# elizabethfong/SparkSmithWaterman

Hardware: NVIDIA B200
Metric: GCUPS incl. traceback (150 bp reads x 10k RefSeq-shaped refs per B200) (higher is better)
Workload: dtype s16x2

## Files before the change

### sparksmithwaterman_b200/csrc/swb_align.cu

```cuda
#include "swb_host.h"

using namespace swbh;

namespace {
struct Segments { std::vector<int32_t> ref, c0, len, skip, end; };
void make_segments(const swb_refset *rs, int K, int match, int mismatch, int gap, bool few_items, Segments &S)
{
    const int64_t m = (int64_t)GL * K;
    const int64_t big = std::max({match, mismatch, 0});
    const int64_t W = m + (big * m) / (-(int64_t)gap) + 1;
    const int64_t W_al = ((W + 8 + 15) / 16) * 16;
    int64_t SEG = few_items ? 1024 : 8192;
    SEG = std::max<int64_t>(SEG, ((2 * W_al + 15) / 16) * 16);
    const int32_t BIG = 1 << 26;
    struct One { int32_t ref, c0, len, skip, end; };
    std::vector<One> v;
    v.reserve((size_t)rs->n_refs + 64);
    for (int64_t s = 0; s < rs->n_refs; ++s) {
        const int64_t n = rs->len_sorted[(size_t)s];
        if (n <= 2 * SEG) { v.push_back(One{(int32_t)s, 0, (int32_t)n, 0, BIG}); continue; }
        const int64_t nseg = (n + SEG - 1) / SEG;
        for (int64_t k = 0; k < nseg; ++k) {
            const int64_t lo = k * SEG, hi = std::min<int64_t>(n, (k + 1) * SEG);
            const int64_t c0 = std::max<int64_t>(0, lo - W_al);
            v.push_back(One{(int32_t)s, (int32_t)c0, (int32_t)(hi - c0), (int32_t)((lo - c0) / CB),
                            k == nseg - 1 ? BIG : (int32_t)((hi - c0) / CB)});
        }
    }
    std::stable_sort(v.begin(), v.end(), [](const One &a, const One &b) { return a.len > b.len; });
    S.ref.clear(); S.c0.clear(); S.len.clear(); S.skip.clear(); S.end.clear();
    for (const One &o : v) { S.ref.push_back(o.ref); S.c0.push_back(o.c0); S.len.push_back(o.len); S.skip.push_back(o.skip); S.end.push_back(o.end); }
}

int pick_k(int m)
{
    for (int k = 0; k < kNumK; ++k)
        if (GL * kKList[k] >= m) return kKList[k];
    return 0;
}

int record_words(int K) { return ((K + 1 + 7) / 8 + CB / 8) * 8; }

using ResultPtr = std::unique_ptr<swb_result, void (*)(swb_result *)>;
ResultPtr new_result(swb_ctx *ctx, const swb_refset *rs, const swb_reads *rd, uint32_t flags)
{
    ResultPtr res(new swb_result(), swb_result_free);
    ctx->live.fetch_add(1);
    res->ctx = ctx; res->n_refs = rs->n_refs; res->n_reads = rd->n_reads; res->flags = flags;
    res->ref_len = rs->len_orig; res->read_len = rd->len;
    int64_t read_bases = 0;
    for (int32_t m : rd->len) read_bases += m;
    res->stats[STAT_CELLS] = (double)rs->total_bases * (double)read_bases;
    res->stats[STAT_PAIRS] = (double)rs->n_refs * (double)rd->n_reads;
    return res;
}
}

struct AlignCall::Batch {
    int n_rp = 0, m_max = 0;
    std::vector<int32_t> h_rp;
    BatchParams P;
};

int AlignCall::run(int32_t *ext_scores, int32_t *ext_totals)
{
    const int64_t n_refs = rs->n_refs, n_reads = rd->n_reads;
    const size_t n_pairs = (size_t)(n_refs * n_reads);
    if (ext_scores) res->d_scores.view(ext_scores, n_pairs); else CU(res->d_scores.alloc(n_pairs, st));
    if (ext_totals) res->d_totals.view(ext_totals, (size_t)n_refs); else CU(res->d_totals.alloc((size_t)n_refs, st));
    CU(res->d_best.alloc((size_t)n_reads * 4, st));
    CU(cudaMemsetAsync(res->d_scores.p, 0, std::max<size_t>(n_pairs, 1) * 4, st));
    res->top_k = top_k; res->min_score = min_score;
    if (top_k > 0) CU(res->d_hits.alloc((size_t)n_reads * top_k * 4, st));

    const auto t_wall0 = std::chrono::steady_clock::now();
    ctx->ev_used = 0;
    CU(ctx->counters.reserve(16, st));
    int rc;
    if (n_refs > 0 && n_reads > 0) {
        std::vector<std::vector<int32_t>> classes(kNumK);
        std::vector<int32_t> wide;
        classify_reads(classes, wide);
        for (int kc = 0; kc < kNumK; ++kc)
            if (!classes[(size_t)kc].empty() && (rc = run_class(kKList[kc], classes[(size_t)kc]))) return rc;
        if (!wide.empty() && (rc = run_wide_reads(wide))) return rc;
    }
    DevBuf<uint32_t> keep;
    if (top_k > 0 && (rc = select_final_hits(keep))) return rc;
    if ((rc = assemble(keep))) return rc;
    return finish_stats(t_wall0);
}

void AlignCall::classify_reads(std::vector<std::vector<int32_t>> &classes, std::vector<int32_t> &wide) const
{
    const bool short_scores_ok = rs->two_bit_ok && gap < 0 && std::abs((int64_t)match) <= 8000 &&
                                 std::abs((int64_t)mismatch) <= 8000 && std::abs((int64_t)gap) <= 8000;
    static const bool no_long = getenv("SWB_NO_LONG_CLASSES") != nullptr;
    const bool long_kernels_ok = !no_long && tile_trace_ok(match, mismatch, gap);
    for (int64_t q = 0; q < rd->n_reads; ++q) {
        const int m = rd->len[(size_t)q];
        if (m == 0) continue;
        const int64_t smax = (int64_t)std::max({match, mismatch, 0}) * std::min<int64_t>(m, rs->max_len);
        const bool is_short = short_scores_ok && smax <= 16000 &&
                              (m <= MAX_SHORT_ROWS || (m <= MAX_LONG_ROWS && long_kernels_ok && fill_bias_ok(match, mismatch, gap, smax)));
        if (!is_short) { wide.push_back((int32_t)q); continue; }
        const int K = pick_k(m);
        for (int k = 0; k < kNumK; ++k) if (kKList[k] == K) classes[(size_t)k].push_back((int32_t)q);
    }
}

int AlignCall::run_class(int K, std::vector<int32_t> &reads)
{
    std::stable_sort(reads.begin(), reads.end(), [&](int32_t a, int32_t b) { return rd->len[(size_t)a] > rd->len[(size_t)b]; });
    const int64_t n_rp_total = ((int64_t)reads.size() + 1) / 2;
    std::shared_ptr<swb_refset::SegTables> segt;
    int rc = seg_tables(K, n_rp_total * ((rs->n_refs + 3) / 4) < (int64_t)ctx->sm_count * 24, segt);
    if (rc) return rc;
    const int64_t bytes_per_rp = rs->blocks_per_rp * ((int64_t)record_words(K) * GL * 4 + GL * 4);
    int64_t rp_per_batch = std::max<int64_t>(1, ctx->ws_bytes / std::max<int64_t>(bytes_per_rp, 1));
    rp_per_batch = std::min<int64_t>(rp_per_batch, 1 << 16);
    if (rp_per_batch * rs->n_refs * 2 >= ((int64_t)1 << 30)) rp_per_batch = std::max<int64_t>(1, (((int64_t)1 << 30) - 1) / (rs->n_refs * 2));
    const int64_t nb = (n_rp_total + rp_per_batch - 1) / rp_per_batch;
    rp_per_batch = (n_rp_total + nb - 1) / nb;
    std::vector<Batch> batches((size_t)nb);
    for (int64_t k = 0; k < nb; ++k) {
        const int64_t rp0 = k * rp_per_batch;
        Batch &b = batches[(size_t)k];
        if ((rc = fill_batch(K, reads, rp0, (int)std::min<int64_t>(rp_per_batch, n_rp_total - rp0), *segt, b))) return rc;
        if ((rc = trace_batch(K, b))) return rc;
    }
    CU(cudaStreamSynchronize(st));
    return SWB_OK;
}

int AlignCall::seg_tables(int K, bool few_items, std::shared_ptr<swb_refset::SegTables> &out)
{
    const swb_refset::SegKey skey{K, match, mismatch, gap, few_items ? 1 : 0};
    auto sit = rs->seg_cache.find(skey);
    if (sit == rs->seg_cache.end()) {
        Segments segs;
        make_segments(rs, K, match, mismatch, gap, few_items, segs);
        auto sc = std::make_shared<swb_refset::SegTables>();
        sc->nv = segs.ref.size();
        CU(sc->ref.alloc(sc->nv, st)); CU(sc->c0.alloc(sc->nv, st)); CU(sc->len.alloc(sc->nv, st));
        CU(sc->skip.alloc(sc->nv, st)); CU(sc->end.alloc(sc->nv, st));
        CU(cudaMemcpyAsync(sc->ref.p, segs.ref.data(), sc->nv * 4, cudaMemcpyHostToDevice, st));
        CU(cudaMemcpyAsync(sc->c0.p, segs.c0.data(), sc->nv * 4, cudaMemcpyHostToDevice, st));
        CU(cudaMemcpyAsync(sc->len.p, segs.len.data(), sc->nv * 4, cudaMemcpyHostToDevice, st));
        CU(cudaMemcpyAsync(sc->skip.p, segs.skip.data(), sc->nv * 4, cudaMemcpyHostToDevice, st));
        CU(cudaMemcpyAsync(sc->end.p, segs.end.data(), sc->nv * 4, cudaMemcpyHostToDevice, st));
        CU(cudaStreamSynchronize(st));
        if (rs->seg_cache.size() >= 16) rs->seg_cache.clear();
        sit = rs->seg_cache.emplace(skey, sc).first;
    }
    out = sit->second;
    return SWB_OK;
}

int AlignCall::fill_batch(int K, const std::vector<int32_t> &reads, int64_t rp0, int n_rp, const swb_refset::SegTables &segt, Batch &b)
{
    b.n_rp = n_rp;
    b.h_rp.assign((size_t)n_rp * 2, -1);
    for (int r = 0; r < n_rp; ++r)
        for (int h = 0; h < 2; ++h) {
            const int64_t x = (rp0 + r) * 2 + h;
            if (x < (int64_t)reads.size()) {
                b.h_rp[(size_t)r * 2 + h] = reads[(size_t)x];
                b.m_max = std::max(b.m_max, rd->len[(size_t)reads[(size_t)x]]);
            }
        }
    ++n_batches;
    CU(ctx->rp.reserve(b.h_rp.size(), st));
    CU(cudaMemcpyAsync(ctx->rp.p, b.h_rp.data(), b.h_rp.size() * 4, cudaMemcpyHostToDevice, st));
    const size_t ck_words = (size_t)n_rp * rs->blocks_per_rp * record_words(K) * GL;
    const size_t tmx_words = (size_t)n_rp * rs->blocks_per_rp * GL;
    CU(ctx->ck.reserve(ck_words, st));
    CU(ctx->tmx.reserve(tmx_words, st));
    ck_bytes += (double)(ck_words + tmx_words) * 4;
    BatchParams &P = b.P;
    P.ref_words = rs->words.p; P.ref_word_off = rs->word_off.p; P.ref_len = rs->len.p;
    P.ref_orig = rs->orig.p; P.ref_sorted_of = rs->sorted_of.p; P.ref_blk_off = rs->blk_off.p;
    P.n_refs = (int32_t)rs->n_refs; P.blocks_per_rp = rs->blocks_per_rp;
    P.v_ref = segt.ref.p; P.v_c0 = segt.c0.p; P.v_len = segt.len.p; P.v_skip = segt.skip.p;
    P.v_end = segt.end.p; P.n_vrefs = (int32_t)segt.nv;
    P.read_codes = rd->codes.p; P.read_off = rd->off.p; P.rp_reads = ctx->rp.p; P.read_slot = nullptr;
    P.n_rp = n_rp; P.n_reads = rd->n_reads;
    P.match = match; P.mismatch = mismatch; P.gap = gap; P.tie_gt = (flags & SWB_F_TIE_GT) ? 1 : 0;
    P.scores = res->d_scores.p; P.rec = ctx->ck.p; P.tmx = ctx->tmx.p; P.sel = nullptr;
    uint32_t *d_work = ctx->counters.p + 4;
    const bool biased = fill_bias_ok(match, mismatch, gap, (int64_t)std::max({match, mismatch, 0}) * std::min<int64_t>(b.m_max, rs->max_len));
    P.seam_bias = biased ? -gap : 0;
    P.tmx_slack = biased ? fill_sub_slack(match, mismatch, gap) : 0;
    CU(timer.begin(STAT_FILL_MS));
    if (biased)
        CU(launch_fill_bias(K, P, d_work, ctx->sm_count, st));
    else
        CU(launch_fill(K, P, d_work, ctx->sm_count, st));
    ++launches;
    CU(timer.end());
    return SWB_OK;
}

int AlignCall::trace_batch(int K, Batch &b)
{
    const bool scores_only = (flags & SWB_F_SCORES_ONLY) != 0;
    size_t sel_words = 0;
    if (top_k > 0 && !scores_only) {
        sel_words = ((size_t)b.n_rp * 2 * (size_t)rs->n_refs + 31) / 32;
        CU(ctx->hit_sel.reserve(sel_words, st));
        b.P.sel = ctx->hit_sel.p;
    }
    const BatchParams &P = b.P;
    if (scores_only && P.tmx_slack == 0) return SWB_OK;
    CU(timer.begin(STAT_LOCATE_MS));
    uint32_t n_cells = 0;
    const int rc = locate_cells(K, b, sel_words, n_cells);
    if (rc) return rc;
    if (scores_only) { CU(timer.end()); return SWB_OK; }
    BatchOut bo;
    bo.n_cells = n_cells;
    CU(bo.keys.alloc(n_cells, st));
    const size_t tmp_bytes = sort_keys_tmp_bytes(n_cells);
    CU(ctx->sort_tmp.reserve(tmp_bytes, st));
    CU(sort_keys(ctx->keys_tmp.p, bo.keys.p, n_cells, ctx->sort_tmp.p, tmp_bytes, st));
    launches += 4;
    CU(timer.end());

    CU(timer.begin(STAT_TRACE_MS));
    const int64_t big = std::max({match, mismatch, 0});
    int64_t lmax = (int64_t)b.m_max + (big * b.m_max - 1) / (-(int64_t)gap) + 1;
    lmax = std::min<int64_t>(lmax, (int64_t)b.m_max + rs->max_len);
    bo.ops_stride = (int)((lmax + 15) / 16);
    CU(bo.beg.alloc(n_cells, st));
    CU(bo.oplen.alloc(n_cells, st));
    CU(bo.ops.alloc((size_t)n_cells * bo.ops_stride, st));
    if (tile_trace_ok(match, mismatch, gap))
        CU(launch_tile_trace(K, P, bo.keys.p, n_cells, bo.beg.p, bo.oplen.p, bo.ops.p, (int)bo.ops_stride, ctx->sm_count, st));
    else
        CU(launch_trace(K, P, bo.keys.p, n_cells, bo.beg.p, bo.oplen.p, bo.ops.p, (int)bo.ops_stride, ctx->sm_count, st));
    ++launches;
    CU(timer.end());
    res->stats[STAT_MAX_CELLS] += n_cells;
    CU(bo.d_slot_read.alloc(b.h_rp.size(), st));
    CU(cudaMemcpyAsync(bo.d_slot_read.p, b.h_rp.data(), b.h_rp.size() * 4, cudaMemcpyHostToDevice, st));
    res->batches.push_back(std::move(bo));
    return SWB_OK;
}

int AlignCall::locate_cells(int K, const Batch &b, size_t sel_words, uint32_t &n_cells)
{
    const BatchParams &P = b.P;
    const bool scores_only = (flags & SWB_F_SCORES_ONLY) != 0;
    uint32_t *d_ntasks = ctx->counters.p, *d_ncells = ctx->counters.p + 1;
    const int64_t pairs_b = (int64_t)b.n_rp * 2 * rs->n_refs;
    uint32_t cap_tasks = (uint32_t)std::min<int64_t>(pairs_b * (P.tmx_slack > 0 ? 4 : 2) + 1024, (int64_t)1 << 31);
    uint32_t cap_cells = (uint32_t)std::min<int64_t>(pairs_b * 2 + 4096, (int64_t)1 << 31);
    uint32_t h_counts[2] = {0, 0};
    for (int attempt = 0; attempt < 3; ++attempt) {
        CU(ctx->tasks.reserve(cap_tasks, st));
        CU(ctx->task_hits.reserve((size_t)cap_tasks * locate_hit_bytes(), st));
        CU(ctx->keys_tmp.reserve(cap_cells, st));
        CU(cudaMemsetAsync(ctx->counters.p, 0, 8, st));
        CU(launch_flag_tiles(P, ctx->tasks.p, cap_tasks, d_ntasks, ctx->sm_count, st));
        CU(launch_locate(K, P, ctx->tasks.p, d_ntasks, cap_tasks, ctx->task_hits.p, ctx->keys_tmp.p, cap_cells, d_ncells,
                         ctx->sm_count, 0, st));
        launches += 2;
        if (sel_words) {
            CU(timer.begin(STAT_SELECT_MS));
            CU(cudaMemsetAsync(ctx->hit_sel.p, 0, sel_words * 4, st));
// ... 458 lines not shown
```

### sparksmithwaterman_b200/csrc/swb_fill_bias.cu

```cuda
#include "swb_internal.h"
#include "swb_device.cuh"

#include <algorithm>
#include <cstdlib>

namespace swb {

__device__ __forceinline__ uint32_t imad_add(uint32_t a, uint32_t one, uint32_t b)
{
    return a * one + b;
}

template <int K>
__device__ __forceinline__ void fill_column(uint32_t (&H)[K], const uint32_t *pcol, uint32_t diag, uint32_t top,
                                            uint32_t floorv, uint32_t g2, uint32_t one)
{
    using G = Geo<K>;
    uint32_t nw = diag, nn = top;
    if constexpr (K <= MAX_K_BASE) {
        uint32_t sv[G::KP];
        load_profile<G::KP>(pcol, sv);
#pragma unroll
        for (int r = 0; r < K; ++r) {
            const uint32_t tt = imad_add(nw, one, sv[r]);
            const uint32_t pre = vmax3(tt, H[r], floorv);
            nw = H[r];
            H[r] = viaddmax(nn, g2, pre);
            nn = H[r];
        }
    } else {
        const uint4 *p4 = reinterpret_cast<const uint4 *>(pcol);
#pragma unroll
        for (int q = 0; q < G::KP / 4; ++q) {
            const uint4 v = p4[q];
            const uint32_t sv[4] = {v.x, v.y, v.z, v.w};
#pragma unroll
            for (int x = 0; x < 4; ++x) {
                const int r = 4 * q + x;
                if (r < K) {
                    const uint32_t tt = imad_add(nw, one, sv[x]);
                    const uint32_t pre = vmax3(tt, H[r < K ? r : 0], floorv);
                    nw = H[r < K ? r : 0];
                    H[r < K ? r : 0] = viaddmax(nn, g2, pre);
                    nn = H[r < K ? r : 0];
                }
            }
        }
    }
}

constexpr int FILL_ROLL_K = 25;
constexpr int fill_bias_threads(int K) { return K <= MAX_K_BASE ? 512 : (K <= 48 ? 384 : 256); }

template <int K, bool SUB>
__global__ void __launch_bounds__(fill_bias_threads(K)) fill_bias_kernel(const BatchParams P, uint32_t *work_counter, uint32_t one)
{
    using G = Geo<K>;
    extern __shared__ __align__(16) uint32_t prof_all[];

    const int lane = threadIdx.x & 31, warp = threadIdx.x >> 5;
    const int t = lane & (GL - 1), g = lane >> 3;
    uint32_t *prof = prof_all + warp * G::PROF_WORDS;
    const int n_quads = (P.n_vrefs + 3) >> 2;
    const uint32_t n_items = (uint32_t)n_quads * (uint32_t)P.n_rp;

    const int ag = -P.gap;
    const uint32_t g2 = pack2(P.gap, P.gap);
    const uint32_t gpos = pack2(ag, ag);
    const uint32_t base_bias = pack2(ag * (8 - t), ag * (8 - t));
    const uint32_t renorm = (uint32_t)(-(int32_t)(pack2(ag * CB, ag * CB)));
    const uint32_t unbias = (uint32_t)(-(int32_t)base_bias);
    const uint32_t negbase = pack2(-ag * (8 - t), -ag * (8 - t));
    const uint32_t g2c = g2 - 0x10000u, g2c2 = 2u * g2c;
    static_assert((CB & 1) == 0, "the subsampled tile maximum tracks the odd steps of a block");
    const int my_prof = t * G::KS;
    int cur_rp = -1, ra = 0, rb = -1;

    for (;;) {
        uint32_t item = 0;
        if (lane == 0) item = atomicAdd(work_counter, 1u);
        item = __shfl_sync(0xffffffffu, item, 0);
        if (item >= n_items) break;
        const int q = (int)(item / (uint32_t)P.n_rp);
        const int rp = (int)(item - (uint32_t)q * (uint32_t)P.n_rp);
        if (rp != cur_rp) {
            cur_rp = rp;
            ra = P.rp_reads[2 * rp]; rb = P.rp_reads[2 * rp + 1];
            const int64_t offa = P.read_off[ra];
            const int ma = (int)(P.read_off[ra + 1] - offa);
            const int64_t offb = rb >= 0 ? P.read_off[rb] : 0;
            const int mb = rb >= 0 ? (int)(P.read_off[rb + 1] - offb) : 0;
            __syncwarp();
            for (int idx = lane; idx < GL * K; idx += 32) {
                const int tt = idx / K, r = idx - tt * K;
                const int row = tt * K + r;
                const int qa = row < ma ? (int)P.read_codes[offa + row] : -1;
                const int qb = row < mb ? (int)P.read_codes[offb + row] : -1;
#pragma unroll
                for (int c = 0; c < 4; ++c) {
                    const int lo = qa < 0 ? 0 : (qa == c ? P.match : P.mismatch) + ag;
                    const int hi = qb < 0 ? 0 : (qb == c ? P.match : P.mismatch) + ag;
                    prof[c * G::CSTRIDE + tt * G::KS + r] = pack2(lo, hi);
                }
            }
            __syncwarp();
        }

        const int v = 4 * q + g;
        const bool has_ref = v < P.n_vrefs;
        const int ref = has_ref ? P.v_ref[v] : 0;
        const int c0 = has_ref ? P.v_c0[v] : 0;
        const int n_g = has_ref ? P.v_len[v] : 0;
        const int skip = has_ref ? P.v_skip[v] : 0;
        const int own_end = has_ref ? P.v_end[v] : 0;
        const int nmax = P.v_len[4 * q];
        const int nmin = (4 * q + 3 < P.n_vrefs) ? P.v_len[4 * q + 3] : 0;
        const uint32_t *wp = P.ref_words + (has_ref ? P.ref_word_off[ref] + (uint32_t)(c0 >> 4) : 0u);
        const int64_t blk0 = (int64_t)rp * P.blocks_per_rp + (has_ref ? P.ref_blk_off[ref] + c0 / CB : 0);
        const int my_steps = has_ref ? min(n_g + GL - 1, own_end * CB) : 0;

        uint32_t H[K];
#pragma unroll
        for (int r = 0; r < K; ++r) H[r] = base_bias;
        uint32_t diag = base_bias, floorv = base_bias, negfloor = negbase;
        uint32_t tmax = 0, gmax = 0, wprev = 0;

        const int nsteps = nmax + GL - 1;
        for (int s0 = 0; s0 < nsteps; s0 += 16) {
            const uint32_t wnew = (s0 < n_g) ? __ldg(wp + (s0 >> 4)) : 0u;
            const uint32_t win = __funnelshift_rc(wprev, wnew, 32 - 2 * t);
            wprev = wnew;
            const bool fast = (s0 >= GL - 1) && (s0 + 16 <= nmin);

            const bool own_chunk = (s0 < my_steps) && ((s0 >> 4) >= skip);
            uint32_t *seam = rec_lane<K>(P.rec, blk0 + (s0 >> 4), t) + G::CKP * REC_P;
            uint32_t tq[8] = {0, 0, 0, 0, 0, 0, 0, 0};

            if (fast) {
                constexpr int UNR = K < FILL_ROLL_K ? 16 : 8;
#pragma unroll 1
                for (int uq = 0; uq < 16; uq += UNR) {
                    const uint32_t winq = win >> (2 * uq);
#pragma unroll
                    for (int uu = 0; uu < UNR; ++uu) {
                        floorv = imad_add(floorv, one, gpos);
                        if (!SUB) negfloor = imad_add(negfloor, one, g2c);
                        uint32_t top = __shfl_up_sync(0xffffffffu, H[K - 1], 1);
                        if (t == 0) top = floorv;
                        const uint32_t c = (winq >> (2 * uu)) & 3u;
                        fill_column<K>(H, prof + c * G::CSTRIDE + my_prof, diag, top, floorv, g2, one);
                        diag = top;
                        if (!SUB) tmax = viaddmax(colmax<K>(floorv, H), negfloor, tmax);
                        else if (uu & 1) {
                            negfloor = imad_add(negfloor, one, g2c2);
                            tmax = viaddmax(colmax_even<K>(floorv, H), negfloor, tmax);
                        }
                        tq[uu & 7] = top;
                        if ((uu & 7) == 7 && own_chunk)
                            stg256(seam + ((uq + uu) >> 3) * REC_P, tq[0], tq[1], tq[2], tq[3], tq[4], tq[5], tq[6], tq[7]);
                    }
                }
            } else {
#pragma unroll 1
                for (int uq = 0; uq < 16; uq += 8) {
#pragma unroll
                    for (int uu = 0; uu < 8; ++uu) {
                        const int u = uq + uu;
                        const int s = s0 + u;
                        floorv = imad_add(floorv, one, gpos);
                        negfloor = imad_add(negfloor, one, g2c);
                        uint32_t top = __shfl_up_sync(0xffffffffu, H[K - 1], 1);
                        if (t == 0) top = floorv;
                        const uint32_t c = (win >> (2 * u)) & 3u;
                        const bool valid = (s >= t) && (s < n_g + t);
                        if (valid) {
                            fill_column<K>(H, prof + c * G::CSTRIDE + my_prof, diag, top, floorv, g2, one);
                            tmax = viaddmax(colmax<K>(floorv, H), negfloor, tmax);
                        } else {
#pragma unroll
                            for (int r = 0; r < K; ++r) H[r] = floorv;
                        }
                        diag = top;
                        tq[uu] = top;
                        if (uu == 7 && own_chunk) stg256(seam + (uq >> 3) * REC_P, tq[0], tq[1], tq[2], tq[3], tq[4], tq[5], tq[6], tq[7]);
                    }
                }
            }

            const int s_next = s0 + 16;
            {
#pragma unroll
                for (int r = 0; r < K; ++r) H[r] = imad_add(H[r], one, renorm);
                diag = imad_add(diag, one, renorm);
                floorv = base_bias;
                negfloor = negbase;
                const int b = s_next / CB;
                if (s_next - CB < my_steps && b - 1 >= skip) {
                    P.tmx[(blk0 + b - 1) * GL + t] = tmax;
                    gmax = vmax2(gmax, tmax);
                }
                tmax = 0;
                if constexpr (K <= MAX_K_BASE) {
                    uint32_t U[K];
#pragma unroll
                    for (int r = 0; r < K; ++r) U[r] = imad_add(H[r], one, unbias);
                    if (s_next < my_steps && b >= skip)
                        store_checkpoint<K>(rec_lane<K>(P.rec, blk0 + b, t), U, imad_add(diag, one, unbias));
                } else if (s_next < my_steps && b >= skip) {
                    uint32_t *lane_rec = rec_lane<K>(P.rec, blk0 + b, t);
#pragma unroll
                    for (int p = 0; p < G::CKP; ++p) {
                        uint32_t v[8];
#pragma unroll
                        for (int e = 0; e < 8; ++e) {
                            const int w = 8 * p + e;
                            v[e] = (w < K) ? imad_add(H[w < K ? w : 0], one, unbias) : (w == K ? imad_add(diag, one, unbias) : 0u);
                        }
                        stg256(lane_rec + p * REC_P, v[0], v[1], v[2], v[3], v[4], v[5], v[6], v[7]);
                    }
                }
            }
        }
        {
            const int s_end = ((nsteps + 15) >> 4) << 4;
            if ((s_end % CB) != 0) {
                const int b_last = s_end / CB;
                if (b_last * CB < my_steps && b_last >= skip) {
                    P.tmx[(blk0 + b_last) * GL + t] = tmax;
                    gmax = vmax2(gmax, tmax);
                }
            }
        }
        gmax = vmax2(gmax, __shfl_xor_sync(0xffffffffu, gmax, 1));
        gmax = vmax2(gmax, __shfl_xor_sync(0xffffffffu, gmax, 2));
        gmax = vmax2(gmax, __shfl_xor_sync(0xffffffffu, gmax, 4));
        if (t == 0 && has_ref) {
            const int64_t ro = P.ref_orig[ref];
            atomicMax(P.scores + ro * P.n_reads + ra, (int)(int16_t)(gmax & 0xffffu));
            if (rb >= 0) atomicMax(P.scores + ro * P.n_reads + rb, (int)(int16_t)(gmax >> 16));
        }
    }
}

template <int K, bool SUB>
static cudaError_t launch_fill_bias_k2(const BatchParams &P, uint32_t *work_counter, int sm_count, cudaStream_t st)
{
    using G = Geo<K>;
    const int n_quads = (P.n_vrefs + 3) / 4;
    static const int env_warps = getenv("SWB_FILL_WARPS") ? atoi(getenv("SWB_FILL_WARPS")) : 0;
    const int max_warps = fill_bias_threads(K) / 32;
    const int warps = std::min(env_warps > 0 ? env_warps : 16, max_warps);
    const int64_t items = (int64_t)n_quads * P.n_rp;
    const int64_t ctas = std::min<int64_t>((items + warps - 1) / warps, (int64_t)sm_count);
    const size_t smem = (size_t)warps * G::PROF_WORDS * sizeof(uint32_t);
    cudaError_t e = cudaSuccess;
    {
        static PerDeviceOnce carve;
        e = carve.run([] { return cudaFuncSetAttribute(fill_bias_kernel<K, SUB>, cudaFuncAttributePreferredSharedMemoryCarveout, cudaSharedmemCarveoutMaxShared); });
        if (e != cudaSuccess) return e;
    }
    if (smem > 48 * 1024) {
        e = cudaFuncSetAttribute(fill_bias_kernel<K, SUB>, cudaFuncAttributeMaxDynamicSharedMemorySize, (int)smem);
        if (e != cudaSuccess) return e;
    }
    e = cudaMemsetAsync(work_counter, 0, sizeof(uint32_t), st);
    if (e != cudaSuccess) return e;
    fill_bias_kernel<K, SUB><<<dim3((unsigned)ctas), dim3(warps * 32), smem, st>>>(P, work_counter, 1u);
    return cudaGetLastError();
}

template <int K>
static cudaError_t launch_fill_bias_k(const BatchParams &P, uint32_t *work_counter, int sm_count, cudaStream_t st)
{
    return P.tmx_slack > 0 ? launch_fill_bias_k2<K, true>(P, work_counter, sm_count, st)
                           : launch_fill_bias_k2<K, false>(P, work_counter, sm_count, st);
}

cudaError_t launch_fill_bias(int K, const BatchParams &P, uint32_t *work_counter, int sm_count, cudaStream_t st)
{
    switch (K) {
        case 4:  return launch_fill_bias_k<4>(P, work_counter, sm_count, st);
        case 5:  return launch_fill_bias_k<5>(P, work_counter, sm_count, st);
        case 7:  return launch_fill_bias_k<7>(P, work_counter, sm_count, st);
        case 10: return launch_fill_bias_k<10>(P, work_counter, sm_count, st);
        case 8:  return launch_fill_bias_k<8>(P, work_counter, sm_count, st);
        case 13: return launch_fill_bias_k<13>(P, work_counter, sm_count, st);
        case 16: return launch_fill_bias_k<16>(P, work_counter, sm_count, st);
        case 19: return launch_fill_bias_k<19>(P, work_counter, sm_count, st);
        case 25: return launch_fill_bias_k<25>(P, work_counter, sm_count, st);
        case 32: return launch_fill_bias_k<32>(P, work_counter, sm_count, st);
        case 40: return launch_fill_bias_k<40>(P, work_counter, sm_count, st);
        case 48: return launch_fill_bias_k<48>(P, work_counter, sm_count, st);
        case 56: return launch_fill_bias_k<56>(P, work_counter, sm_count, st);
        case 64: return launch_fill_bias_k<64>(P, work_counter, sm_count, st);
    }
    return cudaErrorInvalidValue;
}

int fill_sub_slack(int match, int mismatch, int gap)
{
    static const bool disabled = getenv("SWB_NO_SUBSAMPLE") != nullptr;
    if (disabled || gap >= 0) return 0;
    const int ag = -gap;
    const int diag = mismatch >= 0 ? 0 : std::min(-mismatch, 2 * ag);
    const int slack = std::max(ag, diag);
    return (match > slack && slack < 4096) ? slack : 0;
}

bool fill_bias_ok(int match, int mismatch, int gap, int64_t max_score)
{
    if (gap >= 0) return false;
    const int ag = -gap;
    static const bool disabled = getenv("SWB_NO_BIAS_FILL") != nullptr;
    return !disabled && match + ag >= 0 && mismatch + ag >= 0 && match + ag <= 4000 && mismatch + ag <= 4000 &&
           max_score + 32LL * ag <= 30000;
}

}
```

### sparksmithwaterman_b200/csrc/swb_internal.h

```cpp
#pragma once

#include <cstdint>
#include <cuda_runtime.h>
#include <mutex>
#include <string>
#include <vector>

#include "../../include/swb200.h"

namespace swb {

constexpr int GL = 8;
constexpr int CB = 16;
constexpr int MAX_SHORT_ROWS = GL * 32;
static_assert(CB == 16, "the fill kernels store one seam quad per 4 steps of a 16-step chunk");

constexpr int kNumK = 14;
constexpr int kKList[kNumK] = {4, 5, 7, 8, 10, 13, 16, 19, 25, 32,
                               40, 48, 56, 64};
constexpr int MAX_K_BASE = 32;
constexpr int MAX_LONG_ROWS = 511;

template <int K> struct Geo {
    static constexpr int KW = ((K + 1 + 3) / 4) * 4;
// ... 3 lines not shown
    static constexpr int KP = ((K + 3) / 4) * 4;
    static constexpr int KS = ((KP / 4) % 2 == 1) ? KP : KP + 4;
    static constexpr int CSTRIDE = GL * KS;
    static constexpr int PROF_WORDS = 4 * CSTRIDE;
    static constexpr int RS = ((K + 1 + 1) / 2) * 2;
    static constexpr int TILE_HALFWORDS = GL * (CB + 1) * RS;
};

constexpr int16_t S_PAD = -16384;

constexpr int KEY_J_BITS = 22, KEY_I_BITS = 9;
__host__ __device__ inline uint64_t make_key(uint64_t p, uint32_t i, uint32_t j)
{ return (p << (KEY_J_BITS + KEY_I_BITS)) | ((uint64_t)i << KEY_J_BITS) | j; }
__host__ __device__ inline uint64_t key_pair(uint64_t k) { return k >> (KEY_J_BITS + KEY_I_BITS); }
__host__ __device__ inline uint32_t key_i(uint64_t k) { return (uint32_t)(k >> KEY_J_BITS) & ((1u << KEY_I_BITS) - 1); }
__host__ __device__ inline uint32_t key_j(uint64_t k) { return (uint32_t)k & ((1u << KEY_J_BITS) - 1); }

struct PerDeviceOnce {
    std::mutex mu;
    bool done[64] = {};
    template <class F> cudaError_t run(F &&f)
    {
        int d = 0;
        if (cudaGetDevice(&d) != cudaSuccess || d < 0 || d >= 64) return f();
        std::lock_guard<std::mutex> lk(mu);
        if (done[d]) return cudaSuccess;
        const cudaError_t e = f();
        if (e == cudaSuccess) done[d] = true;
        return e;
    }
};

struct TileTask { uint32_t rp_half; uint32_t ref_sorted; uint32_t block; uint32_t lane; };

struct BatchParams {
    const uint32_t *ref_words;
    const uint32_t *ref_word_off;
    const int32_t  *ref_len;
    const int32_t  *ref_orig;
    const int32_t  *ref_sorted_of;
    const int64_t  *ref_blk_off;
    int32_t n_refs;
    int64_t blocks_per_rp;
    const int32_t *v_ref, *v_c0, *v_len, *v_skip, *v_end;
    int32_t n_vrefs;
    const uint8_t *read_codes;
    const int64_t *read_off;
    const int32_t *rp_reads;
    const int32_t *read_slot;
    int32_t n_rp;
    int64_t n_reads;
    int32_t match, mismatch, gap;
    int32_t tie_gt;
    int32_t  *scores;
    uint32_t *rec;
    uint32_t *tmx;
    int32_t tmx_slack;
    int32_t seam_bias;
    const uint32_t *sel;
};

namespace wide {
constexpr int WL = 32;
constexpr int WCB = 32;
constexpr int kNumKL = 3;
constexpr int kKLList[kNumKL] = {8, 16, 32};
template <int KL> struct WGeo {
    static constexpr int BH = WL * KL;
    static constexpr int KW = ((KL + 1 + 3) / 4) * 4;
    static constexpr int RW = KW + WCB;
};
constexpr int wide_rw(int kl) { return ((kl + 1 + 3) / 4) * 4 + WCB; }
__host__ __device__ inline uint64_t wide_key(uint64_t pair, uint32_t i, uint32_t j) { return (pair << 43) | ((uint64_t)i << 22) | j; }
__host__ __device__ inline uint64_t wide_key_pair(uint64_t k) { return k >> 43; }
__host__ __device__ inline uint32_t wide_key_i(uint64_t k) { return (uint32_t)(k >> 22) & ((1u << 21) - 1); }
__host__ __device__ inline uint32_t wide_key_j(uint64_t k) { return (uint32_t)k & ((1u << 22) - 1); }
}

struct WideTask { int32_t pair, band, block; uint32_t lane; };

struct WideParams {
    int32_t n_pairs;
    const int32_t *pair_ref;
    const int32_t *pair_read;
    const uint8_t *ref_codes;
    const int64_t *ref_off;
    const uint8_t *rpad;
    const int64_t *rpad_off;
    const int64_t *read_off;
    int32_t match, mismatch, gap;
    int32_t tie_gt;
    int32_t n_symbols;
    int64_t n_reads;
    const int64_t *band_off;
    const int64_t *blk_off;
    const int64_t *brow_off;
    int32_t *brow;
    int32_t *rec;
    int32_t *tmx;
    int32_t *scores;
    int32_t *mail;
    int32_t *mail_latest;
    int32_t mail_stride;
    int32_t pipe_c;
    unsigned long long *dbg;
};

struct BatchDesc {
    const uint64_t *keys; const int32_t *beg; const int32_t *oplen; const uint32_t *ops;
    const int32_t *slot_read;
    const int64_t *pair_map;
    int64_t ops_stride;
    uint32_t base;
    uint32_t n_cells;
    int32_t wide;
};
size_t      assemble_tmp_bytes(uint32_t n_cells);
cudaError_t assemble_sort(const BatchDesc *batches, int nb, uint32_t n_cells, int64_t n_refs, int64_t n_reads,
                          const uint32_t *keep, uint64_t *pair_tmp, uint32_t *src_tmp, uint64_t *pair_sorted, uint32_t *order, void *tmp,
                          size_t tmp_bytes, int pair_bits, cudaStream_t st);
cudaError_t assemble_gather_cells(const BatchDesc *batches, int nb, uint32_t n_cells, const uint32_t *order, int32_t *cells,
                                  int32_t *beginnings, int32_t *op_lens, int64_t *words, int64_t *ops_off, void *tmp,
                                  size_t tmp_bytes, cudaStream_t st);
cudaError_t assemble_gather_ops(const BatchDesc *batches, int nb, uint32_t n_cells, const uint32_t *order,
                                const int64_t *ops_off, uint32_t *ops_out, cudaStream_t st);
cudaError_t assemble_offsets(const uint64_t *pair_sorted, uint32_t n_cells, int64_t n_pairs, int64_t *cell_off,
                             int32_t *best, int64_t n_reads, const int32_t *cells, cudaStream_t st);

cudaError_t assemble_kept_count(const uint64_t *pair_sorted, uint32_t n_cells, int64_t n_pairs, uint32_t *n_kept, cudaStream_t st);
cudaError_t assemble_hit_cells(const BatchDesc *batches, int nb, const uint64_t *pair_sorted, const uint32_t *order, uint32_t n_all,
                               int64_t n_pairs, int64_t n_reads, const int64_t *cell_off, const int32_t *cells, int32_t *best,
                               int32_t *hits, int k, cudaStream_t st);

size_t      select_hits_tmp_elems(int64_t n_refs, int64_t n_slots, int k);
cudaError_t launch_select_hits(const int32_t *scores, int64_t n_refs, int64_t n_reads, const int32_t *slots, int64_t n_slots,
                               int k, int32_t min_score, int with_best, int4 *hits, uint32_t *bits, int64_t bit_slot,
                               int64_t bit_ref, uint64_t *tmp, size_t tmp_elems, cudaStream_t st);

cudaError_t launch_wide_pad_reads(const uint8_t *codes, const int64_t *read_off, const int32_t *reads, int n_reads,
                                  const int64_t *rpad_off, const int64_t *rpad_len, uint8_t *rpad, int64_t max_len,
                                  cudaStream_t st);
cudaError_t launch_wide_fill(int KL, const WideParams &P, const int2 *items, int n_items, uint32_t *ticket, int sm_count,
                             cudaStream_t st);
cudaError_t launch_wide_flag(const WideParams &P, int64_t total_blocks, WideTask *tasks, uint32_t cap, uint32_t *count,
                             int sm_count, cudaStream_t st);
cudaError_t launch_wide_locate(int KL, const WideParams &P, const WideTask *tasks, const uint32_t *n_tasks, uint32_t cap_tasks,
                               uint64_t *keys, uint32_t cap, uint32_t *count, int sm_count, cudaStream_t st);
cudaError_t launch_wide_trace(int KL, const WideParams &P, const uint64_t *keys, uint32_t n_cells, int32_t *beginnings,
                              int32_t *op_lens, uint32_t *ops, int64_t ops_stride, int sm_count, cudaStream_t st);

cudaError_t launch_fill(int K, const BatchParams &P, uint32_t *work_counter, int sm_count, cudaStream_t st);
cudaError_t launch_fill_bias(int K, const BatchParams &P, uint32_t *work_counter, int sm_count, cudaStream_t st);
bool fill_bias_ok(int match, int mismatch, int gap, int64_t max_score);
int fill_sub_slack(int match, int mismatch, int gap);
cudaError_t launch_flag_tiles(const BatchParams &P, TileTask *tasks, uint32_t cap, uint32_t *count, int sm_count, cudaStream_t st);
cudaError_t launch_locate(int K, const BatchParams &P, const TileTask *tasks, const uint32_t *n_tasks,
                          uint32_t cap_tasks, void *hits, uint64_t *keys, uint32_t cap, uint32_t *count, int sm_count,
                          int phase, cudaStream_t st);
size_t      locate_hit_bytes();
cudaError_t launch_trace(int K, const BatchParams &P, const uint64_t *keys, uint32_t n_cells,
                         int32_t *beginnings, int32_t *op_lens, uint32_t *ops, int ops_stride_words,
                         int sm_count, cudaStream_t st);
cudaError_t launch_tile_trace(int K, const BatchParams &P, const uint64_t *keys, uint32_t n_cells,
                              int32_t *beginnings, int32_t *op_lens, uint32_t *ops, int ops_stride_words,
                              int sm_count, cudaStream_t st);
bool tile_trace_ok(int match, int mismatch, int gap);
cudaError_t launch_cell_offsets(const uint64_t *keys, uint32_t n_cells, const int64_t *pair_ids, int64_t n_pairs,
                                int64_t *offsets, cudaStream_t st);
cudaError_t launch_ref_totals(const int32_t *scores, int64_t n_refs, int64_t n_reads, int32_t *totals, cudaStream_t st);
cudaError_t launch_best_hits(const int32_t *scores, int64_t n_refs, int64_t n_reads, int32_t *best, int sm_count, cudaStream_t st);
cudaError_t sort_keys(uint64_t *keys_in, uint64_t *keys_out, uint32_t n, void *tmp, size_t tmp_bytes, cudaStream_t st);
size_t      sort_keys_tmp_bytes(uint32_t n);

}
```

Measured before the change: 9920.

## Process two read pairs per lane in bias fill kernel for small K

The bias fill kernel now processes RPL=2 read pairs per warp work item when K is below the roll threshold. Each reference column's encoding, floor and negfloor bookkeeping and shuffle loop structure are then shared across two independent DP chains, which raises instruction-level parallelism and amortises per-column overhead. The cost is doubled register state for H, a per-warp profile in shared memory twice as large, and a lower thread cap of 384. The host segment-table heuristic is adjusted to count work units instead of read pairs.

Result: slower. 8852 (median of 6 runs) (-10.8%).

```diff
diff --git a/sparksmithwaterman_b200/csrc/swb_align.cu b/sparksmithwaterman_b200/csrc/swb_align.cu
--- a/sparksmithwaterman_b200/csrc/swb_align.cu
+++ b/sparksmithwaterman_b200/csrc/swb_align.cu
@@ -113,8 +113,10 @@
 {
     std::stable_sort(reads.begin(), reads.end(), [&](int32_t a, int32_t b) { return rd->len[(size_t)a] > rd->len[(size_t)b]; });
     const int64_t n_rp_total = ((int64_t)reads.size() + 1) / 2;
+    const int64_t smax = (int64_t)std::max({match, mismatch, 0}) * std::min<int64_t>(rd->len[(size_t)reads[0]], rs->max_len);
+    const int rpl = fill_bias_ok(match, mismatch, gap, smax) ? fill_bias_pairs_per_lane(K) : 1;
     std::shared_ptr<swb_refset::SegTables> segt;
-    int rc = seg_tables(K, n_rp_total * ((rs->n_refs + 3) / 4) < (int64_t)ctx->sm_count * 24, segt);
+    int rc = seg_tables(K, (n_rp_total + rpl - 1) / rpl * ((rs->n_refs + 3) / 4) < (int64_t)ctx->sm_count * 24, segt);
     if (rc) return rc;
     const int64_t bytes_per_rp = rs->blocks_per_rp * ((int64_t)record_words(K) * GL * 4 + GL * 4);
     int64_t rp_per_batch = std::max<int64_t>(1, ctx->ws_bytes / std::max<int64_t>(bytes_per_rp, 1));
diff --git a/sparksmithwaterman_b200/csrc/swb_fill_bias.cu b/sparksmithwaterman_b200/csrc/swb_fill_bias.cu
--- a/sparksmithwaterman_b200/csrc/swb_fill_bias.cu
+++ b/sparksmithwaterman_b200/csrc/swb_fill_bias.cu
@@ -11,38 +11,44 @@
     return a * one + b;
 }
 
-template <int K>
-__device__ __forceinline__ void fill_column(uint32_t (&H)[K], const uint32_t *pcol, uint32_t diag, uint32_t top,
-                                            uint32_t floorv, uint32_t g2, uint32_t one)
+__device__ __forceinline__ void fill_cell(uint32_t &h, uint32_t &nw, uint32_t &nn, uint32_t s, uint32_t floorv, uint32_t g2,
+                                          uint32_t one)
+{
+    const uint32_t tt = imad_add(nw, one, s);
+    const uint32_t pre = vmax3(tt, h, floorv);
+    nw = h;
+    h = viaddmax(nn, g2, pre);
+    nn = h;
+}
+
+template <int K, int RPL>
+__device__ __forceinline__ void fill_column(uint32_t (&H)[RPL][K], const uint32_t *pcol, const uint32_t (&diag)[RPL],
+                                            const uint32_t (&top)[RPL], uint32_t floorv, uint32_t g2, uint32_t one)
 {
     using G = Geo<K>;
-    uint32_t nw = diag, nn = top;
-    if constexpr (K <= MAX_K_BASE) {
+    uint32_t nw[RPL], nn[RPL];
+#pragma unroll
+    for (int p = 0; p < RPL; ++p) { nw[p] = diag[p]; nn[p] = top[p]; }
+    if constexpr (K <= MAX_K_BASE && RPL == 1) {
         uint32_t sv[G::KP];
         load_profile<G::KP>(pcol, sv);
 #pragma unroll
-        for (int r = 0; r < K; ++r) {
-            const uint32_t tt = imad_add(nw, one, sv[r]);
-            const uint32_t pre = vmax3(tt, H[r], floorv);
-            nw = H[r];
-            H[r] = viaddmax(nn, g2, pre);
-            nn = H[r];
-        }
+        for (int r = 0; r < K; ++r) fill_cell(H[0][r], nw[0], nn[0], sv[r], floorv, g2, one);
     } else {
-        const uint4 *p4 = reinterpret_cast<const uint4 *>(pcol);
 #pragma unroll
         for (int q = 0; q < G::KP / 4; ++q) {
-            const uint4 v = p4[q];
-            const uint32_t sv[4] = {v.x, v.y, v.z, v.w};
+            uint32_t sv[RPL][4];
+#pragma unroll
+            for (int p = 0; p < RPL; ++p) {
+                const uint4 v = reinterpret_cast<const uint4 *>(pcol + p * G::PROF_WORDS)[q];
+                sv[p][0] = v.x; sv[p][1] = v.y; sv[p][2] = v.z; sv[p][3] = v.w;
+            }
 #pragma unroll
             for (int x = 0; x < 4; ++x) {
                 const int r = 4 * q + x;
                 if (r < K) {
-                    const uint32_t tt = imad_add(nw, one, sv[x]);
-                    const uint32_t pre = vmax3(tt, H[r < K ? r : 0], floorv);
-                    nw = H[r < K ? r : 0];
-                    H[r < K ? r : 0] = viaddmax(nn, g2, pre);
-                    nn = H[r < K ? r : 0];
+#pragma unroll
+                    for (int p = 0; p < RPL; ++p) fill_cell(H[p][r < K ? r : 0], nw[p], nn[p], sv[p][x], floorv, g2, one);
                 }
             }
         }
@@ -50,19 +56,20 @@
 }
 
 constexpr int FILL_ROLL_K = 25;
-constexpr int fill_bias_threads(int K) { return K <= MAX_K_BASE ? 512 : (K <= 48 ? 384 : 256); }
-
-template <int K, bool SUB>
-__global__ void __launch_bounds__(fill_bias_threads(K)) fill_bias_kernel(const BatchParams P, uint32_t *work_counter, uint32_t one)
+constexpr int fill_bias_threads(int K, int RPL) { return K <= MAX_K_BASE ? (RPL == 2 ? 384 : 512) : (K <= 48 ? 384 : 256); }
+
+template <int K, bool SUB, int RPL>
+__global__ void __launch_bounds__(fill_bias_threads(K, RPL)) fill_bias_kernel(const BatchParams P, uint32_t *work_counter, uint32_t one)
 {
     using G = Geo<K>;
     extern __shared__ __align__(16) uint32_t prof_all[];
 
     const int lane = threadIdx.x & 31, warp = threadIdx.x >> 5;
     const int t = lane & (GL - 1), g = lane >> 3;
-    uint32_t *prof = prof_all + warp * G::PROF_WORDS;
+    uint32_t *prof = prof_all + warp * (RPL * G::PROF_WORDS);
     const int n_quads = (P.n_vrefs + 3) >> 2;
-    const uint32_t n_items = (uint32_t)n_quads * (uint32_t)P.n_rp;
+    const int n_units = (P.n_rp + RPL - 1) / RPL;
+    const uint32_t n_items = (uint32_t)n_quads * (uint32_t)n_units;
 
     const int ag = -P.gap;
     const uint32_t g2 = pack2(P.gap, P.gap);
@@ -74,33 +81,41 @@
     const uint32_t g2c = g2 - 0x10000u, g2c2 = 2u * g2c;
     static_assert((CB & 1) == 0, "the subsampled tile maximum tracks the odd steps of a block");
     const int my_prof = t * G::KS;
-    int cur_rp = -1, ra = 0, rb = -1;
+    int cur_unit = -1, np = 0, ra[RPL], rb[RPL];
+#pragma unroll
+    for (int p = 0; p < RPL; ++p) { ra[p] = 0; rb[p] = -1; }
 
     for (;;) {
         uint32_t item = 0;
         if (lane == 0) item = atomicAdd(work_counter, 1u);
         item = __shfl_sync(0xffffffffu, item, 0);
         if (item >= n_items) break;
-        const int q = (int)(item / (uint32_t)P.n_rp);
-        const int rp = (int)(item - (uint32_t)q * (uint32_t)P.n_rp);
-        if (rp != cur_rp) {
-            cur_rp = rp;
-            ra = P.rp_reads[2 * rp]; rb = P.rp_reads[2 * rp + 1];
-            const int64_t offa = P.read_off[ra];
-            const int ma = (int)(P.read_off[ra + 1] - offa);
-            const int64_t offb = rb >= 0 ? P.read_off[rb] : 0;
-            const int mb = rb >= 0 ? (int)(P.read_off[rb + 1] - offb) : 0;
+        const int q = (int)(item / (uint32_t)n_units);
+        const int unit = (int)(item - (uint32_t)q * (uint32_t)n_units);
+        if (unit != cur_unit) {
+            cur_unit = unit;
+            np = min(RPL, P.n_rp - unit * RPL);
             __syncwarp();
-            for (int idx = lane; idx < GL * K; idx += 32) {
-                const int tt = idx / K, r = idx - tt * K;
-                const int row = tt * K + r;
-                const int qa = row < ma ? (int)P.read_codes[offa + row] : -1;
-                const int qb = row < mb ? (int)P.read_codes[offb + row] : -1;
-#pragma unroll
-                for (int c = 0; c < 4; ++c) {
-                    const int lo = qa < 0 ? 0 : (qa == c ? P.match : P.mismatch) + ag;
-                    const int hi = qb < 0 ? 0 : (qb == c ? P.match : P.mismatch) + ag;
-                    prof[c * G::CSTRIDE + tt * G::KS + r] = pack2(lo, hi);
+#pragma unroll
+            for (int p = 0; p < RPL; ++p) {
+                const int rp = unit * RPL + p;
+                ra[p] = p < np ? P.rp_reads[2 * rp] : -1; rb[p] = p < np ? P.rp_reads[2 * rp + 1] : -1;
+                const int64_t offa = ra[p] >= 0 ? P.read_off[ra[p]] : 0;
+                const int ma = ra[p] >= 0 ? (int)(P.read_off[ra[p] + 1] - offa) : 0;
+                const int64_t offb = rb[p] >= 0 ? P.read_off[rb[p]] : 0;
+                const int mb = rb[p] >= 0 ? (int)(P.read_off[rb[p] + 1] - offb) : 0;
+                uint32_t *pprof = prof + p * G::PROF_WORDS;
+                for (int idx = lane; idx < GL * K; idx += 32) {
+                    const int tt = idx / K, r = idx - tt * K;
+                    const int row = tt * K + r;
+                    const int qa = row < ma ? (int)P.read_codes[offa + row] : -1;
+                    const int qb = row < mb ? (int)P.read_codes[offb + row] : -1;
+#pragma unroll
+                    for (int c = 0; c < 4; ++c) {
+                        const int lo = qa < 0 ? 0 : (qa == c ? P.match : P.mismatch) + ag;
+                        const int hi = qb < 0 ? 0 : (qb == c ? P.match : P.mismatch) + ag;
+                        pprof[c * G::CSTRIDE + tt * G::KS + r] = pack2(lo, hi);
+                    }
                 }
             }
             __syncwarp();
@@ -116,14 +131,20 @@
         const int nmax = P.v_len[4 * q];
         const int nmin = (4 * q + 3 < P.n_vrefs) ? P.v_len[4 * q + 3] : 0;
         const uint32_t *wp = P.ref_words + (has_ref ? P.ref_word_off[ref] + (uint32_t)(c0 >> 4) : 0u);
-        const int64_t blk0 = (int64_t)rp * P.blocks_per_rp + (has_ref ? P.ref_blk_off[ref] + c0 / CB : 0);
+        int64_t blk0[RPL];
+#pragma unroll
+        for (int p = 0; p < RPL; ++p)
+            blk0[p] = (int64_t)(unit * RPL + p) * P.blocks_per_rp + (has_ref ? P.ref_blk_off[ref] + c0 / CB : 0);
         const int my_steps = has_ref ? min(n_g + GL - 1, own_end * CB) : 0;
 
-        uint32_t H[K];
-#pragma unroll
-        for (int r = 0; r < K; ++r) H[r] = base_bias;
-        uint32_t diag = base_bias, floorv = base_bias, negfloor = negbase;
-        uint32_t tmax = 0, gmax = 0, wprev = 0;
+        uint32_t H[RPL][K], diag[RPL], tmax[RPL], gmax[RPL];
+#pragma unroll
+        for (int p = 0; p < RPL; ++p) {
+#pragma unroll
+            for (int r = 0; r < K; ++r) H[p][r] = base_bias;
+            diag[p] = base_bias; tmax[p] = 0; gmax[p] = 0;
+        }
+        uint32_t floorv = base_bias, negfloor = negbase, wprev = 0;
 
         const int nsteps = nmax + GL - 1;
         for (int s0 = 0; s0 < nsteps; s0 += 16) {
@@ -133,8 +154,10 @@
             const bool fast = (s0 >= GL - 1) && (s0 + 16 <= nmin);
 
             const bool own_chunk = (s0 < my_steps) && ((s0 >> 4) >= skip);
-            uint32_t *seam = rec_lane<K>(P.rec, blk0 + (s0 >> 4), t) + G::CKP * REC_P;
-            uint32_t tq[8] = {0, 0, 0, 0, 0, 0, 0, 0};
+            uint32_t *seam[RPL];
+#pragma unroll
+            for (int p = 0; p < RPL; ++p) seam[p] = rec_lane<K>(P.rec, blk0[p] + (s0 >> 4), t) + G::CKP * REC_P;
+            uint32_t tq[RPL][8] = {};
 
             if (fast) {
                 constexpr int UNR = K < FILL_ROLL_K ? 16 : 8;
@@ -145,19 +168,26 @@
                     for (int uu = 0; uu < UNR; ++uu) {
                         floorv = imad_add(floorv, one, gpos);
                         if (!SUB) negfloor = imad_add(negfloor, one, g2c);
-                        uint32_t top = __shfl_up_sync(0xffffffffu, H[K - 1], 1);
-                        if (t == 0) top = floorv;
+                        uint32_t top[RPL];
+#pragma unroll
+                        for (int p = 0; p < RPL; ++p) {
+                            top[p] = __shfl_up_sync(0xffffffffu, H[p][K - 1], 1);
+                            if (t == 0) top[p] = floorv;
+                        }
                         const uint32_t c = (winq >> (2 * uu)) & 3u;
-                        fill_column<K>(H, prof + c * G::CSTRIDE + my_prof, diag, top, floorv, g2, one);
-                        diag = top;
-                        if (!SUB) tmax = viaddmax(colmax<K>(floorv, H), negfloor, tmax);
-                        else if (uu & 1) {
-                            negfloor = imad_add(negfloor, one, g2c2);
-                            tmax = viaddmax(colmax_even<K>(floorv, H), negfloor, tmax);
-                        }
-                        tq[uu & 7] = top;
-                        if ((uu & 7) == 7 && own_chunk)
-                            stg256(seam + ((uq + uu) >> 3) * REC_P, tq[0], tq[1], tq[2], tq[3], tq[4], tq[5], tq[6], tq[7]);
+                        fill_column<K, RPL>(H, prof + c * G::CSTRIDE + my_prof, diag, top, floorv, g2, one);
+                        if (SUB && (uu & 1)) negfloor = imad_add(negfloor, one, g2c2);
+#pragma unroll
+                        for (int p = 0; p < RPL; ++p) {
+                            diag[p] = top[p];
+                            if (!SUB) tmax[p] = viaddmax(colmax<K>(floorv, H[p]), negfloor, tmax[p]);
+                            else if (uu & 1)
+                                tmax[p] = viaddmax(colmax_even<K>(floorv, H[p]), negfloor, tmax[p]);
+                            tq[p][uu & 7] = top[p];
+                            if ((uu & 7) == 7 && own_chunk && p < np)
+                                stg256(seam[p] + ((uq + uu) >> 3) * REC_P, tq[p][0], tq[p][1], tq[p][2], tq[p][3], tq[p][4],
+                                       tq[p][5], tq[p][6], tq[p][7]);
+                        }
                     }
                 }
             } else {
@@ -169,111 +199,135 @@
                         const int s = s0 + u;
                         floorv = imad_add(floorv, one, gpos);
                         negfloor = imad_add(negfloor, one, g2c);
-                        uint32_t top = __shfl_up_sync(0xffffffffu, H[K - 1], 1);
-                        if (t == 0) top = floorv;
+                        uint32_t top[RPL];
+#pragma unroll
+                        for (int p = 0; p < RPL; ++p) {
+                            top[p] = __shfl_up_sync(0xffffffffu, H[p][K - 1], 1);
+                            if (t == 0) top[p] = floorv;
+                        }
                         const uint32_t c = (win >> (2 * u)) & 3u;
                         const bool valid = (s >= t) && (s < n_g + t);
                         if (valid) {
-                            fill_column<K>(H, prof + c * G::CSTRIDE + my_prof, diag, top, floorv, g2, one);
-                            tmax = viaddmax(colmax<K>(floorv, H), negfloor, tmax);
+                            fill_column<K, RPL>(H, prof + c * G::CSTRIDE + my_prof, diag, top, floorv, g2, one);
+#pragma unroll
+                            for (int p = 0; p < RPL; ++p) tmax[p] = viaddmax(colmax<K>(floorv, H[p]), negfloor, tmax[p]);
                         } else {
 #pragma unroll
-                            for (int r = 0; r < K; ++r) H[r] = floorv;
-                        }
-                        diag = top;
-                        tq[uu] = top;
-                        if (uu == 7 && own_chunk) stg256(seam + (uq >> 3) * REC_P, tq[0], tq[1], tq[2], tq[3], tq[4], tq[5], tq[6], tq[7]);
+                            for (int p = 0; p < RPL; ++p)
+#pragma unroll
+                                for (int r = 0; r < K; ++r) H[p][r] = floorv;
+                        }
+#pragma unroll
+                        for (int p = 0; p < RPL; ++p) {
+                            diag[p] = top[p];
+                            tq[p][uu] = top[p];
+                            if (uu == 7 && own_chunk && p < np)
+                                stg256(seam[p] + (uq >> 3) * REC_P, tq[p][0], tq[p][1], tq[p][2], tq[p][3], tq[p][4], tq[p][5],
+                                       tq[p][6], tq[p][7]);
+                        }
                     }
                 }
             }
 
             const int s_next = s0 + 16;
-            {
-#pragma unroll
-                for (int r = 0; r < K; ++r) H[r] = imad_add(H[r], one, renorm);
-                diag = imad_add(diag, one, renorm);
-                floorv = base_bias;
-                negfloor = negbase;
-                const int b = s_next / CB;
-                if (s_next - CB < my_steps && b - 1 >= skip) {
-                    P.tmx[(blk0 + b - 1) * GL + t] = tmax;
-                    gmax = vmax2(gmax, tmax);
-                }
-                tmax = 0;
+            floorv = base_bias;
+            negfloor = negbase;
+            const int b = s_next / CB;
+#pragma unroll
+            for (int p = 0; p < RPL; ++p) {
+#pragma unroll
+                for (int r = 0; r < K; ++r) H[p][r] = imad_add(H[p][r], one, renorm);
+                diag[p] = imad_add(diag[p], one, renorm);
+                if (s_next - CB < my_steps && b - 1 >= skip && p < np) {
+                    P.tmx[(blk0[p] + b - 1) * GL + t] = tmax[p];
+                    gmax[p] = vmax2(gmax[p], tmax[p]);
+                }
+                tmax[p] = 0;
                 if constexpr (K <= MAX_K_BASE) {
                     uint32_t U[K];
 #pragma unroll
-                    for (int r = 0; r < K; ++r) U[r] = imad_add(H[r], one, unbias);
-                    if (s_next < my_steps && b >= skip)
-                        store_checkpoint<K>(rec_lane<K>(P.rec, blk0 + b, t), U, imad_add(diag, one, unbias));
-                } else if (s_next < my_steps && b >= skip) {
-                    uint32_t *lane_rec = rec_lane<K>(P.rec, blk0 + b, t);
-#pragma unroll
-                    for (int p = 0; p < G::CKP; ++p) {
+                    for (int r = 0; r < K; ++r) U[r] = imad_add(H[p][r], one, unbias);
+                    if (s_next < my_steps && b >= skip && p < np)
+                        store_checkpoint<K>(rec_lane<K>(P.rec, blk0[p] + b, t), U, imad_add(diag[p], one, unbias));
+                } else if (s_next < my_steps && b >= skip && p < np) {
+                    uint32_t *lane_rec = rec_lane<K>(P.rec, blk0[p] + b, t);
+#pragma unroll
+                    for (int pc = 0; pc < G::CKP; ++pc) {
                         uint32_t v[8];
 #pragma unroll
                         for (int e = 0; e < 8; ++e) {
-                            const int w = 8 * p + e;
-                            v[e] = (w < K) ? imad_add(H[w < K ? w : 0], one, unbias) : (w == K ? imad_add(diag, one, unbias) : 0u);
-                        }
-                        stg256(lane_rec + p * REC_P, v[0], v[1], v[2], v[3], v[4], v[5], v[6], v[7]);
+                            const int w = 8 * pc + e;
+                            v[e] = (w < K) ? imad_add(H[p][w < K ? w : 0], one, unbias) : (w == K ? imad_add(diag[p], one, unbias) : 0u);
+                        }
+                        stg256(lane_rec + pc * REC_P, v[0], v[1], v[2], v[3], v[4], v[5], v[6], v[7]);
                     }
                 }
             }
         }
-        {
-            const int s_end = ((nsteps + 15) >> 4) << 4;
-            if ((s_end % CB) != 0) {
-                const int b_last = s_end / CB;
-                if (b_last * CB < my_steps && b_last >= skip) {
-                    P.tmx[(blk0 + b_last) * GL + t] = tmax;
-                    gmax = vmax2(gmax, tmax);
-                }
-            }
-        }
-        gmax = vmax2(gmax, __shfl_xor_sync(0xffffffffu, gmax, 1));
-        gmax = vmax2(gmax, __shfl_xor_sync(0xffffffffu, gmax, 2));
-        gmax = vmax2(gmax, __shfl_xor_sync(0xffffffffu, gmax, 4));
-        if (t == 0 && has_ref) {
-            const int64_t ro = P.ref_orig[ref];
-            atomicMax(P.scores + ro * P.n_reads + ra, (int)(int16_t)(gmax & 0xffffu));
-            if (rb >= 0) atomicMax(P.scores + ro * P.n_reads + rb, (int)(int16_t)(gmax >> 16));
-        }
-    }
-}
-
-template <int K, bool SUB>
+        const int s_end = ((nsteps + 15) >> 4) << 4;
+        const int b_last = s_end / CB;
+        const bool last_tile = (s_end % CB) != 0 && b_last * CB < my_steps && b_last >= skip;
+#pragma unroll
+        for (int p = 0; p < RPL; ++p) {
+            if (last_tile && p < np) {
+                P.tmx[(blk0[p] + b_last) * GL + t] = tmax[p];
+                gmax[p] = vmax2(gmax[p], tmax[p]);
+            }
+            gmax[p] = vmax2(gmax[p], __shfl_xor_sync(0xffffffffu, gmax[p], 1));
+            gmax[p] = vmax2(gmax[p], __shfl_xor_sync(0xffffffffu, gmax[p], 2));
+            gmax[p] = vmax2(gmax[p], __shfl_xor_sync(0xffffffffu, gmax[p], 4));
+            if (t == 0 && has_ref && p < np) {
+                const int64_t ro = P.ref_orig[ref];
+                atomicMax(P.scores + ro * P.n_reads + ra[p], (int)(int16_t)(gmax[p] & 0xffffu));
+                if (rb[p] >= 0) atomicMax(P.scores + ro * P.n_reads + rb[p], (int)(int16_t)(gmax[p] >> 16));
+            }
+        }
+    }
+}
+
+template <int K, bool SUB, int RPL>
 static cudaError_t launch_fill_bias_k2(const BatchParams &P, uint32_t *work_counter, int sm_count, cudaStream_t st)
 {
     using G = Geo<K>;
     const int n_quads = (P.n_vrefs + 3) / 4;
     static const int env_warps = getenv("SWB_FILL_WARPS") ? atoi(getenv("SWB_FILL_WARPS")) : 0;
-    const int max_warps = fill_bias_threads(K) / 32;
+    const int max_warps = fill_bias_threads(K, RPL) / 32;
     const int warps = std::min(env_warps > 0 ? env_warps : 16, max_warps);
-    const int64_t items = (int64_t)n_quads * P.n_rp;
+    const int64_t items = (int64_t)n_quads * ((P.n_rp + RPL - 1) / RPL);
     const int64_t ctas = std::min<int64_t>((items + warps - 1) / warps, (int64_t)sm_count);
-    const size_t smem = (size_t)warps * G::PROF_WORDS * sizeof(uint32_t);
+    const size_t smem = (size_t)warps * RPL * G::PROF_WORDS * sizeof(uint32_t);
     cudaError_t e = cudaSuccess;
     {
         static PerDeviceOnce carve;
-        e = carve.run([] { return cudaFuncSetAttribute(fill_bias_kernel<K, SUB>, cudaFuncAttributePreferredSharedMemoryCarveout, cudaSharedmemCarveoutMaxShared); });
+        e = carve.run([] { return cudaFuncSetAttribute(fill_bias_kernel<K, SUB, RPL>, cudaFuncAttributePreferredSharedMemoryCarveout, cudaSharedmemCarveoutMaxShared); });
         if (e != cudaSuccess) return e;
     }
     if (smem > 48 * 1024) {
-        e = cudaFuncSetAttribute(fill_bias_kernel<K, SUB>, cudaFuncAttributeMaxDynamicSharedMemorySize, (int)smem);
+        e = cudaFuncSetAttribute(fill_bias_kernel<K, SUB, RPL>, cudaFuncAttributeMaxDynamicSharedMemorySize, (int)smem);
         if (e != cudaSuccess) return e;
     }
     e = cudaMemsetAsync(work_counter, 0, sizeof(uint32_t), st);
     if (e != cudaSuccess) return e;
-    fill_bias_kernel<K, SUB><<<dim3((unsigned)ctas), dim3(warps * 32), smem, st>>>(P, work_counter, 1u);
+    fill_bias_kernel<K, SUB, RPL><<<dim3((unsigned)ctas), dim3(warps * 32), smem, st>>>(P, work_counter, 1u);
     return cudaGetLastError();
+}
+
+int fill_bias_pairs_per_lane(int K)
+{
+    static const bool one_pair = getenv("SWB_FILL_ONE_PAIR") != nullptr;
+    return (K < FILL_ROLL_K && !one_pair) ? 2 : 1;
 }
 
 template <int K>
 static cudaError_t launch_fill_bias_k(const BatchParams &P, uint32_t *work_counter, int sm_count, cudaStream_t st)
 {
-    return P.tmx_slack > 0 ? launch_fill_bias_k2<K, true>(P, work_counter, sm_count, st)
-                           : launch_fill_bias_k2<K, false>(P, work_counter, sm_count, st);
+    if constexpr (K < FILL_ROLL_K) {
+        if (fill_bias_pairs_per_lane(K) == 2)
+            return P.tmx_slack > 0 ? launch_fill_bias_k2<K, true, 2>(P, work_counter, sm_count, st)
+                                   : launch_fill_bias_k2<K, false, 2>(P, work_counter, sm_count, st);
+    }
+    return P.tmx_slack > 0 ? launch_fill_bias_k2<K, true, 1>(P, work_counter, sm_count, st)
+                           : launch_fill_bias_k2<K, false, 1>(P, work_counter, sm_count, st);
 }
 
 cudaError_t launch_fill_bias(int K, const BatchParams &P, uint32_t *work_counter, int sm_count, cudaStream_t st)
diff --git a/sparksmithwaterman_b200/csrc/swb_internal.h b/sparksmithwaterman_b200/csrc/swb_internal.h
--- a/sparksmithwaterman_b200/csrc/swb_internal.h
+++ b/sparksmithwaterman_b200/csrc/swb_internal.h
@@ -179,6 +179,7 @@
 cudaError_t launch_fill(int K, const BatchParams &P, uint32_t *work_counter, int sm_count, cudaStream_t st);
 cudaError_t launch_fill_bias(int K, const BatchParams &P, uint32_t *work_counter, int sm_count, cudaStream_t st);
 bool fill_bias_ok(int match, int mismatch, int gap, int64_t max_score);
+int fill_bias_pairs_per_lane(int K);
 int fill_sub_slack(int match, int mismatch, int gap);
 cudaError_t launch_flag_tiles(const BatchParams &P, TileTask *tasks, uint32_t cap, uint32_t *count, int sm_count, cudaStream_t st);
 cudaError_t launch_locate(int K, const BatchParams &P, const TileTask *tasks, const uint32_t *n_tasks,
```
